# zhoubin-me/agent0

Hardware: AMD Instinct MI355X
Metric: env-frames/sec (learner FPS: transitions collected and saved to replay per second with the learner running, pre-frameskip) (higher is better)
Workload: dtype f32

## Files before the change

### agent0_amd/csrc/encoder_fused.hip

```cpp
#include "a0_internal.h"
#include "net_tables.h"
#include "operands.h"
#include "update_tail.h"

#include <cstdlib>
#include <type_traits>

typedef float a0_acc4 __attribute__((ext_vector_type(4)));

struct a0_fused_args {
    const uint8_t* frames; const int* slot; long long sample_stride; int chan_off;
    const float *wt1, *wt2, *wt3;
    const float *wx2, *wx3;
    const float *b1, *b2, *b3;
    float *act1, *act2, *act3;
    int B;
    int C, H, W, H1, W1, H2, W2, H3, W3;
    int off_act1, off_act2, off_end;
    int rp1, rp2;
};

A0_HD void a0_fused_set_wt(a0_fused_args& P, const float* wt, int C) {
    const a0_wt_layout T{C};
    P.wt1 = wt + T.conv1x(); P.wt2 = wt + T.conv2(); P.wt3 = wt + T.conv3(); P.wx2 = wt + T.conv2x(); P.wx3 = wt + T.conv3x();
// ... 405 lines not shown
        for (int i = 0; i < HB0; ++i)
            if (h * HB0 + i < MBT) {
#pragma unroll
                for (int t = 0; t < 3; ++t) a[slot][i][t] = *(const uint4*)(af.planes + rows[h * HB0 + i] + off + t * AFX::term);
            }
    };
    fetch(0, 0, af.step_off(wk));
    __builtin_amdgcn_s_waitcnt(0x0F70);
#pragma unroll 1
    for (int tb = 0; tb < NSTW; tb += R) {
#pragma unroll
        for (int u = 0; u < R; ++u) {
            const int st = wk + WK * (tb + u);
            const int off = af.step_off(st), offn = af.step_off(tb + u + 1 < NSTW ? st + WK : st);
#pragma unroll
            for (int h = 0; h < 2; ++h) {
                if (h == 0) fetch(1, 1, off);
                else fetch(0, 0, offn);
                __builtin_amdgcn_sched_barrier(0);
#pragma unroll
                for (int ta = 0; ta < 3; ++ta)
#pragma unroll
                    for (int tw = 0; tw < 3; ++tw)
#pragma unroll
                        for (int i = 0; i < HB0; ++i) {
                            if (ta + tw > ORD || h * HB0 + i >= MBT) continue;
                            const a0_u32x4 av = {a[h][i][ta].x, a[h][i][ta].y, a[h][i][ta].z, a[h][i][ta].w};
                            const a0_u32x4 bv = {ring.v[u][0][tw].x, ring.v[u][0][tw].y, ring.v[u][0][tw].z, ring.v[u][0][tw].w};
                            acc[h * HB0 + i] = __builtin_amdgcn_mfma_f32_16x16x32_bf16(__builtin_bit_cast(a0_bf16x8, bv), __builtin_bit_cast(a0_bf16x8, av), acc[h * HB0 + i], 0, 0, 0);
                        }
                __builtin_amdgcn_sched_barrier(0);
            }
            ring.fill(u);
            __builtin_amdgcn_sched_barrier(0);
        }
    }
    between();
    a0_acc4* x0 = (a0_acc4*)xch0;
    a0_acc4* x1 = (a0_acc4*)xch1;
    constexpr int P1 = (HB1 - 1) * 64 + 4 * LR;
    const int last = q * LR + r16;
    const int n0 = wn * 16 + 4 * q;
    float pe[EPI::PER_ELEM ? HB0 : 1][4];
    auto send = [&](auto mine) {
        constexpr int H = decltype(mine)::value;
        if constexpr (EPI::PER_ELEM) {
#pragma unroll
            for (int i = 0; i < (H == 0 ? HB0 : HB1); ++i) {
                const int m = (H * HB0 + i) * 16 + r16;
                const a0_f4 v = epi.pre_elem4(m < M ? m : M - 1, n0);
                pe[i][0] = v.x; pe[i][1] = v.y; pe[i][2] = v.z; pe[i][3] = v.w;
            }
        }
        if constexpr (H == 1) {
#pragma unroll
            for (int i = 0; i < HB0; ++i) x0[(wn * HB0 + i) * 64 + lane] = acc[i];
        } else {
#pragma unroll
            for (int i = 0; i < HB1; ++i) {
                if (i < HB1 - 1) x1[wn * P1 + i * 64 + lane] = acc[HB0 + i];
                else if (r16 < LR) x1[wn * P1 + (HB1 - 1) * 64 + last] = acc[HB0 + i];
            }
        }
    };
    auto recv = [&](auto mine) {
        constexpr int H = decltype(mine)::value;
#pragma unroll
        for (int i = 0; i < (H == 0 ? HB0 : HB1); ++i) {
            const int mb = H * HB0 + i;
            const int m = mb * 16 + r16;
            if constexpr (H == 0) acc[mb] += x0[(wn * HB0 + i) * 64 + lane];
            else {
                if (i < HB1 - 1) acc[mb] += x1[wn * P1 + i * 64 + lane];
                else if (r16 < LR) acc[mb] += x1[wn * P1 + (HB1 - 1) * 64 + last];
            }
            if (mb < MB && m < M) epi.emit_n4(m, n0, acc[mb], EPI::PER_ELEM ? pe[EPI::PER_ELEM ? i : 0] : nullptr);
        }
    };
    if (wk == 0) send(std::integral_constant<int, 0>{});
    else send(std::integral_constant<int, 1>{});
    __syncthreads();
    if (wk == 0) recv(std::integral_constant<int, 0>{});
    else recv(std::integral_constant<int, 1>{});
    __syncthreads();
}
constexpr int A0_P1X = 40, A0_P2X = 80;
constexpr int A0_RP1X = 20 * A0_P1X + 8;
constexpr int A0_RP2X = 9 * A0_P2X + 96;

constexpr int A0_R1 = 4, A0_R2 = 4, A0_R3 = 6;

template <int MBW1, int MBW2, int MBW3, int WC, bool X9, bool LOOP = false, int ORD = 4>
__global__ __launch_bounds__(A0_FUSED_THREADS) void a0_encoder_fused_kernel(a0_fused_args P);

constexpr int A0_X9_BIAS_OFF = 2 * 4 * 84 * 84 + 3 * 20 * A0_RP1X * 2;
constexpr int A0_RK2 = 2, A0_RK3 = 3;
constexpr int A0_X9_XCH0 = 3 * 9 * A0_RP2X * 2;
constexpr int A0_X9_XCH1 = A0_X9_BIAS_OFF + 160 * 4;
static_assert(A0_X9_XCH0 + 4 * 3 * 1024 <= 2 * 4 * 84 * 84, "conv2 exchange region 0 fits into the image");
constexpr int A0_X9_LDS_BYTES = A0_X9_XCH1 + 4 * (2 * 64 + 4) * 16;
static_assert(A0_X9_LDS_BYTES <= 160 * 1024, "LDS");
static_assert(A0_FUSED_WAVES == 8, "N-stationary stages: four waves along N, two along K");
typedef a0_wring9<64, 4, A0_RK2, 2> a0_ring2_t;
typedef a0_wring9<64, 4, A0_RK3, 2> a0_ring3_t;
template <int ORD, bool LOOP>
A0_D void a0_x9_conv23(const a0_fused_args& P, int b, unsigned char* smem, float* bias_lds, a0_wring1<A0_R1>& ring1, a0_ring2_t& ring2, a0_ring3_t& ring3) {
    const int obs_bytes = P.C * P.H * P.W;
    const int M2 = P.H2 * P.W2, M3 = P.H3 * P.W3;
    uint16_t* a1p = (uint16_t*)(smem + 2 * obs_bytes);
    constexpr int term1 = 20 * A0_RP1X, term2 = 9 * A0_RP2X;
    uint16_t* a2p = (uint16_t*)smem;
    typedef EpiFwdX<9, A0_P2X, A0_RP2X, term2> E2X;
    const AF2X<term1> f2{a1p, A0_RP1X, P.W2, A0_P1X};
    const E2X e2{bias_lds + 32, a2p, P.act2 ? P.act2 + (long long)b * M2 * 64 : nullptr, 64};
    const AF3X<term2> f3{a2p, A0_RP2X, P.W3, A0_P2X};
    const EpiFwdT e3{bias_lds + 96, P.act3 + (long long)b * M3 * 64, 64};
    a0_conv_stage_x9k<ORD, 64, 4, 6, A0_RK2, 1>(f2, M2, ring2, e2, (float*)(smem + A0_X9_XCH0), (float*)(smem + A0_X9_XCH1), [&] { ring3.prologue(); });
    a0_conv_stage_x9k<ORD, 64, 4, 4, A0_RK3, 16>(f3, M3, ring3, e3, (float*)a1p, (float*)a1p + 4 * 2 * 256, [&] { if (LOOP) ring1.prologue(); });
}

A0_D void a0_bytes16_to_img(uint16_t* img, int idx16, const uint4& v) {
    const uint32_t w[4] = {v.x, v.y, v.z, v.w};
    uint32_t o[8];
#pragma unroll
    for (int k = 0; k < 4; ++k) {
        const uint32_t f0 = __float_as_uint((float)(w[k] & 0xffu)), f1 = __float_as_uint((float)((w[k] >> 8) & 0xffu));
        const uint32_t f2 = __float_as_uint((float)((w[k] >> 16) & 0xffu)), f3 = __float_as_uint((float)(w[k] >> 24));
        o[2 * k] = __builtin_amdgcn_perm(f1, f0, 0x07060302u);
        o[2 * k + 1] = __builtin_amdgcn_perm(f3, f2, 0x07060302u);
    }
    ((uint4*)img)[2 * idx16] = uint4{o[0], o[1], o[2], o[3]};
    ((uint4*)img)[2 * idx16 + 1] = uint4{o[4], o[5], o[6], o[7]};
}

template <int ORD, bool LOOP>
A0_D void a0_encoder_fused_x9_body(const a0_fused_args& P, int bid, int nblk) {
    extern __shared__ __attribute__((aligned(16))) unsigned char smem[];
    uint16_t* img = (uint16_t*)smem;
    const int obs_bytes = P.C * P.H * P.W;
    const int M1 = P.H1 * P.W1;
    uint16_t* a1p = (uint16_t*)(smem + 2 * obs_bytes);
    constexpr int term1 = 20 * A0_RP1X;
    typedef EpiFwdX<20, A0_P1X, A0_RP1X, term1> E1X;
    a0_wring1<A0_R1> ring1;
    a0_ring2_t ring2;
    a0_ring3_t ring3;
    ring1.init(P.wt1, P.C);
    ring2.init(P.wx2, 512);
    ring3.init(P.wx3, 576);
    ring1.prologue();
    constexpr int MBW1X = (25 + A0_WMG1 - 1) / A0_WMG1;
    a0_pre<32, 2, MBW1X, E1X> pre1;
    float* bias_lds = (float*)(smem + A0_X9_BIAS_OFF);
    if (threadIdx.x < 160) bias_lds[threadIdx.x] = threadIdx.x < 32 ? P.b1[threadIdx.x] : threadIdx.x < 96 ? P.b2[threadIdx.x - 32] : P.b3[threadIdx.x - 96];
    for (int b = bid; b < P.B; b += nblk) {
        const long long s = P.slot ? (long long)P.slot[b] : (long long)b;
        const uint4* src = (const uint4*)(P.frames + s * P.sample_stride + P.chan_off);
        constexpr int TRIPS = 4;
        const int n16 = obs_bytes >> 4;
        for (int i0 = threadIdx.x; i0 < n16; i0 += TRIPS * A0_FUSED_THREADS) {
            uint4 v[TRIPS];
#pragma unroll
            for (int j = 0; j < TRIPS; ++j) {
                const int i = i0 + j * A0_FUSED_THREADS;
                v[j] = src[i < n16 ? i : n16 - 1];
            }
#pragma unroll
            for (int j = 0; j < TRIPS; ++j) {
                const int i = i0 + j * A0_FUSED_THREADS;
                a0_bytes16_to_img(img, i < n16 ? i : n16 - 1, v[j]);
            }
        }
        __syncthreads();
        const E1X e1{bias_lds, a1p, P.act1 ? P.act1 + (long long)b * M1 * 32 : nullptr, 32};
        const int wmg1 = __builtin_amdgcn_readfirstlane(threadIdx.x >> 6) / 2;
        if (MBW1X > 1 && wmg1 + (MBW1X - 1) * A0_WMG1 >= ((M1 + 15) >> 4))
            a0_conv1_stage<(MBW1X > 1 ? MBW1X - 1 : 1), A0_R1, 84>(img, P.H * P.W, P.W, P.W1, M1, ring1, e1, pre1, [&] { ring2.prologue(); });
        else
            a0_conv1_stage<MBW1X, A0_R1, 84>(img, P.H * P.W, P.W, P.W1, M1, ring1, e1, pre1, [&] { ring2.prologue(); });
        a0_x9_conv23<ORD, LOOP>(P, b, smem, bias_lds, ring1, ring2, ring3);
        if constexpr (!LOOP) break;
    }
}

#include "actor_tail.h"
struct a0_step_enc_args { const float *wt, *b1, *b2, *b3; float* act3; };
template <int ORD>
__global__ __launch_bounds__(A0_FUSED_THREADS) void a0_actor_dist_step_enc_kernel(a0_dtenv_args Q, a0_step_enc_args N) {
    __shared__ int s_chase_cell;
    extern __shared__ __attribute__((aligned(16))) unsigned char smem[];
    unsigned long long v_wt = (unsigned long long)N.wt, v_b1 = (unsigned long long)N.b1, v_b2 = (unsigned long long)N.b2, v_b3 = (unsigned long long)N.b3,
                       v_a3 = (unsigned long long)N.act3, v_obs = (unsigned long long)Q.obs_out;
    A0_TO_VGPR(v_wt); A0_TO_VGPR(v_b1); A0_TO_VGPR(v_b2); A0_TO_VGPR(v_b3); A0_TO_VGPR(v_a3); A0_TO_VGPR(v_obs);
    int v_E = Q.E;
    A0_TO_VGPR(v_E);
    a0_actor_dist_tail_env_body(Q, (float*)smem, &s_chase_cell);
    __syncthreads();
    auto uni = [](unsigned long long v) {
        return ((unsigned long long)(unsigned)__builtin_amdgcn_readfirstlane((int)(v >> 32)) << 32) | (unsigned long long)(unsigned)__builtin_amdgcn_readfirstlane((int)(v & 0xffffffffull));
    };
    const float* wt = (const float*)uni(v_wt);
    a0_fused_args P;
    P.frames = (const uint8_t*)uni(v_obs); P.slot = nullptr; P.sample_stride = 4 * 84 * 84; P.chan_off = 0;
    a0_fused_set_wt(P, wt, 4);
    P.b1 = (const float*)uni(v_b1); P.b2 = (const float*)uni(v_b2); P.b3 = (const float*)uni(v_b3);
    P.act1 = nullptr; P.act2 = nullptr; P.act3 = (float*)uni(v_a3); P.B = __builtin_amdgcn_readfirstlane(v_E);
    P.C = 4; P.H = 84; P.W = 84; P.H1 = 20; P.W1 = 20; P.H2 = 9; P.W2 = 9; P.H3 = 7; P.W3 = 7;
    P.off_act1 = 0; P.off_act2 = 0; P.off_end = 0; P.rp1 = 0; P.rp2 = 0;
    a0_encoder_fused_x9_body<ORD, false>(P, (int)blockIdx.x, (int)gridDim.x);
}

template <int MBW, class EPI, class Mid, class Between>
A0_D void a0_conv1_stage_split(const uint16_t* img, a0_wring1<A0_R1>& ring, const EPI& epi, bool first_before_mid, Mid&& mid, Between&& between) {
    static_assert(A0_R1 == 4 && EPI::TR, "ring of four steps, transposed accumulators");
    constexpr int HW = 84 * 84, W = 84, W1 = 20, M = 400, MB = 25;
// ... 186 lines not shown
        if (has_group()) {
#pragma unroll
            for (int c = 0; c < 4; ++c) row16[c * G16] = keep[c];
            const int nc = !chase ? 4 : (!term ? 3 : 0);
#pragma unroll
            for (int c = 0; c < 4; ++c)
                if (c < nc) { out16[c * G16] = keep[4 + c]; row16[(4 + c) * G16] = keep[4 + c]; }
        }
    };
    auto mid = [&] {
        if (wave != 0) early_stores();
        __syncthreads();
        if (chase) {
            if (has_group()) {
                uint32_t by, bx;
                a0_chase_pos(s_chase_cell, by, bx);
                const uint4 nw = new_group(by, bx);
                if (term) { put(0, nw); put(1, nw); put(2, nw); }
                put(3, nw);
            }
            __syncthreads();
        }
    };
    auto uni = [](unsigned long long v) {
        return ((unsigned long long)(unsigned)__builtin_amdgcn_readfirstlane((int)(v >> 32)) << 32) | (unsigned long long)(unsigned)__builtin_amdgcn_readfirstlane((int)(v & 0xffffffffull));
    };
    ring2.init((const float*)uni(v_wx2), 512);
    ring3.init((const float*)uni(v_wx3), 576);
    typedef EpiFwdX<20, A0_P1X, A0_RP1X, 20 * A0_RP1X> E1X;
    const E1X e1{bias_lds, a1p, nullptr, 32};
    constexpr int MBW1X = (25 + A0_WMG1 - 1) / A0_WMG1;
    const bool before = early && wave != 0;
    if (MBW1X > 1 && wave / 2 + (MBW1X - 1) * A0_WMG1 >= 25)
        a0_conv1_stage_split<(MBW1X > 1 ? MBW1X - 1 : 1)>(img, ring1, e1, before, mid, [&] { ring2.prologue(); });
    else
        a0_conv1_stage_split<MBW1X>(img, ring1, e1, before, mid, [&] { ring2.prologue(); });
    P.act3 = (float*)uni((unsigned long long)act3_v);
    a0_x9_conv23<ORD, false>(P, (int)e, smem, bias_lds, ring1, ring2, ring3);
}

template <int ORD>
__global__ __launch_bounds__(A0_FUSED_THREADS) void a0_actor_step_enc2_kernel(a0_qenv_args Q, a0_step_enc_args N) { a0_actor_step_enc2_body<ORD, TailScalar>(Q, N); }

static bool a0_fused_layout(int C, int H, int W, a0_fused_args& P, size_t& lds_bytes);
int a0_actor_dist_step_enc_launch(const a0_dtenv_args& Q, size_t tail_lds, const float* wt, const a0_encoder_weights* w, float* act3, hipStream_t st) {
    a0_fused_args P;
    size_t lds = 0;
    if (!wt || !w || !w->b1 || !w->b2 || !w->b3 || !act3 || !a0_fused_layout(4, 84, 84, P, lds)) return a0_fail(A0_EINVAL, "a0_actor_dist_tail_env_step_enc: bad encoder argument");
    if (P.H1 != 20 || P.W1 != 20 || P.H2 != 9 || P.W2 != 9 || P.H3 != 7 || P.W3 != 7) return a0_fail(A0_EINVAL, "a0_actor_dist_tail_env_step_enc: geometry");
    const a0_step_enc_args N{wt, w->b1, w->b2, w->b3, act3};
    lds = A0_X9_LDS_BYTES > tail_lds ? (size_t)A0_X9_LDS_BYTES : tail_lds;
    if (lds > 160 * 1024 - 64) return a0_fail(A0_EINVAL, "a0_actor_dist_tail_env_step_enc: head too wide for LDS");
    const int six = a0_x9_products_now() == 6;
    auto kern = six ? a0_actor_dist_step_enc_kernel<2> : a0_actor_dist_step_enc_kernel<4>;
    static size_t configured[2] = {0, 0};
    if (lds > configured[six]) {
        if (hipFuncSetAttribute((const void*)kern, hipFuncAttributeMaxDynamicSharedMemorySize, (int)lds) != hipSuccess)
            return a0_fail(A0_EINVAL, "a0_actor_dist_tail_env_step_enc: LDS");
        configured[six] = lds;
    }
    A0_LAUNCH_PROBED(A0_TAG_ACTOR_STEP_ENC, 2.0 * (400.0 * 32 * 256 + 81.0 * 64 * 512 + 49.0 * 64 * 576) * Q.E, kern, dim3(Q.E), dim3(A0_FUSED_THREADS), lds, st, Q, N);
    return a0_fail_hip((int)hipGetLastError(), "a0_actor_dist_tail_env_step_enc");
}
int a0_actor_step_enc_launch(const a0_qenv_args& Q, const float* wt, const a0_encoder_weights* w, float* act3, hipStream_t st) {
    a0_fused_args P;
    size_t lds = 0;
    if (!wt || !w || !w->b1 || !w->b2 || !w->b3 || !act3 || !a0_fused_layout(4, 84, 84, P, lds)) return a0_fail(A0_EINVAL, "a0_actor_qhead_env_step_enc: bad encoder argument");
    if (P.H1 != 20 || P.W1 != 20 || P.H2 != 9 || P.W2 != 9 || P.H3 != 7 || P.W3 != 7) return a0_fail(A0_EINVAL, "a0_actor_qhead_env_step_enc: geometry");
    const a0_step_enc_args N{wt, w->b1, w->b2, w->b3, act3};
    const size_t tail_lds = (size_t)(Q.A + (Q.dueling ? 1 : 0)) * 512 * sizeof(float);
    lds = A0_X9_LDS_BYTES > tail_lds ? (size_t)A0_X9_LDS_BYTES : tail_lds;
    const int six = a0_x9_products_now() == 6;
    auto kern = six ? a0_actor_step_enc2_kernel<2> : a0_actor_step_enc2_kernel<4>;
    static size_t configured[2] = {0, 0};
    if (lds > configured[six]) {
        if (hipFuncSetAttribute((const void*)kern, hipFuncAttributeMaxDynamicSharedMemorySize, (int)lds) != hipSuccess)
            return a0_fail(A0_EINVAL, "a0_actor_qhead_env_step_enc: LDS");
        configured[six] = lds;
    }
    A0_LAUNCH_PROBED(A0_TAG_ACTOR_STEP_ENC, 2.0 * (400.0 * 32 * 256 + 81.0 * 64 * 512 + 49.0 * 64 * 576) * Q.E, kern, dim3(Q.E), dim3(A0_FUSED_THREADS), lds, st, Q, N);
    return a0_fail_hip((int)hipGetLastError(), "a0_actor_qhead_env_step_enc");
}

struct a0_fused_multi_args { a0_fused_args p[3]; int first[4]; };
template <int ORD>
__global__ __launch_bounds__(A0_FUSED_THREADS) void a0_encoder_fused_multi_kernel(a0_fused_multi_args M) {
    const int bid = (int)blockIdx.x;
    const int k = bid >= M.first[2] ? 2 : (bid >= M.first[1] ? 1 : 0);
    a0_encoder_fused_x9_body<ORD, true>(M.p[k], bid - M.first[k], M.first[k + 1] - M.first[k]);
}

template <int MBW1, int MBW2, int MBW3, int WC, bool X9, bool LOOP, int ORD>
__global__ __launch_bounds__(A0_FUSED_THREADS) void a0_encoder_fused_kernel(a0_fused_args P) {
    if constexpr (X9) {
        static_assert(MBW1 == 7 && MBW2 == 3 && MBW3 == 2 && WC == 84, "the split-operand body is written for the 4 x 84 x 84 geometry");
        a0_encoder_fused_x9_body<ORD, LOOP>(P, (int)blockIdx.x, (int)gridDim.x);
        return;
    }
    extern __shared__ __attribute__((aligned(16))) unsigned char smem[];
    uint16_t* img = (uint16_t*)smem;
    float* fl = (float*)smem;
    float* act1 = fl + P.off_act1;
    float* act2 = fl + P.off_act2;
    const int obs_bytes = P.C * P.H * P.W;
    const int M1 = P.H1 * P.W1, M2 = P.H2 * P.W2, M3 = P.H3 * P.W3;
    a0_wring1<A0_R1> ring1;
    a0_wring<64, 4, A0_R2> ring2;
    a0_wring<64, 4, A0_R3> ring3;
    ring1.init(P.wt1, P.C);
    ring2.init(P.wt2, 512);
    ring3.init(P.wt3, 576);
    ring1.prologue();
    constexpr int OW1 = WC == 84 ? 20 : 0, OW2 = WC == 84 ? 9 : 0;
    a0_pre<32, 2, MBW1, EpiFwd<OW1>> pre1;
    a0_pre<64, 4, MBW2, EpiFwd<OW2>> pre2;
    a0_pre<64, 4, MBW3, EpiFwd<0>> pre3;
    pre1.load(EpiFwd<OW1>{P.b1, nullptr, 0, 0, 1, nullptr, 32}, M1);
    pre2.load(EpiFwd<OW2>{P.b2, nullptr, 0, 0, 1, nullptr, 64}, M2);
    pre3.load(EpiFwd<0>{P.b3, nullptr, 0, 0, 1, nullptr, 64}, M3);
    for (int b = blockIdx.x; b < P.B; b += gridDim.x) {
        const long long s = P.slot ? (long long)P.slot[b] : (long long)b;
        const uint4* src = (const uint4*)(P.frames + s * P.sample_stride + P.chan_off);
        constexpr int TRIPS = 4;
        const int n16 = obs_bytes >> 4;
        for (int i0 = threadIdx.x; i0 < n16; i0 += TRIPS * A0_FUSED_THREADS) {
            uint4 v[TRIPS];
#pragma unroll
            for (int j = 0; j < TRIPS; ++j) {
                const int i = i0 + j * A0_FUSED_THREADS;
                v[j] = src[i < n16 ? i : n16 - 1];
            }
#pragma unroll
            for (int j = 0; j < TRIPS; ++j) {
                const int i = i0 + j * A0_FUSED_THREADS;
                a0_bytes16_to_img(img, i < n16 ? i : n16 - 1, v[j]);
            }
        }
        __syncthreads();
        const EpiFwd<OW1> e1{P.b1, act1, A0_P1, P.rp1, P.W1, P.act1 ? P.act1 + (long long)b * M1 * 32 : nullptr, 32};
        const int wmg1 = __builtin_amdgcn_readfirstlane(threadIdx.x >> 6) / 2;
        if (MBW1 > 1 && wmg1 + (MBW1 - 1) * 4 >= ((M1 + 15) >> 4))
            a0_conv1_stage<(MBW1 > 1 ? MBW1 - 1 : 1), A0_R1, WC>(img, P.H * P.W, P.W, P.W1, M1, ring1, e1, pre1, [&] { ring2.prologue(); });
        else
            a0_conv1_stage<MBW1, A0_R1, WC>(img, P.H * P.W, P.W, P.W1, M1, ring1, e1, pre1, [&] { ring2.prologue(); });
        AF2 f2{act1, P.rp1, P.W2};
        const EpiFwd<OW2> e2{P.b2, act2, A0_P2, P.rp2, P.W2, P.act2 ? P.act2 + (long long)b * M2 * 64 : nullptr, 64};
        a0_conv_stage<64, 4, MBW2, 3, A0_R2>(f2, M2, 512, ring2, e2, pre2, [&] { ring3.prologue(); });
        AF3 f3{act2, P.rp2, P.W3};
        const EpiFwd<0> e3{P.b3, nullptr, 0, 0, 1, P.act3 + (long long)b * M3 * 64, 64};
        a0_conv_stage<64, 4, MBW3, 3, A0_R3>(f3, M3, 576, ring3, e3, pre3, [&] { ring1.prologue(); });
    }
}

struct a0_dgrad_args {
    const float *d3, *act1, *act2;
    float *d2, *d1;
    const float *wd3, *wd2;
    int B;
};
constexpr int A0_RPDA = 11 * A0_P2X + 96, A0_RPDB = 11 * A0_P2X + 48;
constexpr int A0_DTERMA = 11 * A0_RPDA, A0_DTERMB = 11 * A0_RPDB;
struct AFD3X {
    static constexpr int term = A0_DTERMA;
    const uint16_t* planes;
    A0_D int row(int m) const { const int oh = m / 9, ow = m - oh * 9; return oh * A0_RPDA + ow * A0_P2X; }
    A0_D int step_off(int st) const { const int tap = st >> 1; return (tap / 3) * A0_RPDA + (tap % 3) * A0_P2X + 32 * (st & 1); }
};
struct AFD2X {
    static constexpr int term = A0_DTERMB;
    const uint16_t* planes;
    A0_D int row(int m) const { const int oh = m / 10, ow = m - oh * 10; return oh * A0_RPDB + ow * A0_P2X; }
    A0_D int step_off(int st) const { const int cell = st >> 1; return (cell >> 1) * A0_RPDB + (cell & 1) * A0_P2X + 32 * (st & 1); }
};
struct EpiBwd3X {
    static constexpr bool PER_ELEM = true;
    static constexpr bool ROW4 = false;
    static constexpr bool TR = true;
    const float* mask; float* dst; uint16_t* planes;
    A0_D a0_f4 pre_elem4(int m, int n0) const { return *(const a0_f4*)(mask + (unsigned)(m * 64 + n0)); }
    A0_D void emit_n4(int m, int n0, const a0_acc4& acc, const float* pre) const {
        float v[4];
#pragma unroll
        for (int r = 0; r < 4; ++r) v[r] = pre[r] > 0.f ? acc[r] : 0.f;
        *(a0_f4*)(dst + (unsigned)(m * 64 + n0)) = a0_f4{v[0], v[1], v[2], v[3]};
        uint2 hi, mid, lo;
        a0_split4(v, hi, mid, lo);
        const int oh = m / 9, ow = m - oh * 9;
        uint16_t* d = planes + (oh + 1) * A0_RPDB + (ow + 1) * A0_P2X + n0;
        *(uint2*)d = hi; *(uint2*)(d + A0_DTERMB) = mid; *(uint2*)(d + 2 * A0_DTERMB) = lo;
    }
};
static_assert((A0_RPDB % 4) == 0 && (A0_DTERMB % 4) == 0 && (A0_P2X % 4) == 0, "8-byte aligned plane writes");
struct EpiBwdPair {
    static constexpr bool PER_ELEM = true;
    static constexpr bool ROW4 = false;
    static constexpr bool TR = true;
    const float* mask; float* dst; int p0;
    A0_D unsigned gi(int m, int n0) const {
        const int p = p0 + (n0 >> 5), oh = m / 10, ow = m - oh * 10;
        return (unsigned)(((oh * 2 + (p >> 1)) * 20 + ow * 2 + (p & 1)) * 32 + (n0 & 31));
    }
    A0_D a0_f4 pre_elem4(int m, int n0) const { return *(const a0_f4*)(mask + gi(m, n0)); }
    A0_D void emit_n4(int m, int n0, const a0_acc4& acc, const float* pre) const {
        *(a0_f4*)(dst + gi(m, n0)) = a0_f4{pre[0] > 0.f ? acc[0] : 0.f, pre[1] > 0.f ? acc[1] : 0.f, pre[2] > 0.f ? acc[2] : 0.f, pre[3] > 0.f ? acc[3] : 0.f};
    }
};
template <int ORD>
__global__ __launch_bounds__(A0_FUSED_THREADS) void a0_encoder_dgrad_fused_x9_kernel(a0_dgrad_args P) {
    extern __shared__ __attribute__((aligned(16))) unsigned char smem[];
    uint16_t* plA = (uint16_t*)smem;
    uint16_t* plB = plA + 3 * A0_DTERMA;
    for (int i = threadIdx.x; i < 3 * (A0_DTERMA + A0_DTERMB) / 2; i += A0_FUSED_THREADS) ((uint32_t*)smem)[i] = 0u;
    float* const xch0 = (float*)(smem + 3 * (A0_DTERMA + A0_DTERMB) * 2);
    float* const xch1 = xch0 + 4 * 4 * 256;
    const int lane = threadIdx.x & 63, wave = __builtin_amdgcn_readfirstlane(threadIdx.x >> 6), wn = wave & 3, wk = wave >> 2;
    a0_wring9<64, 4, 3, 2> ring3;
    a0_wring9<64, 4, 2, 2> ringq[2];
    ring3.init(P.wd3, 576);
    ring3.prologue();
    const uint4* const wq = (const uint4*)P.wd2 + (((wn & 1) * 16 + (lane & 15)) * 4 + (lane >> 4)) * 3 + (wn >> 1) * 3072 + wk * 384;
    __syncthreads();
    for (int b = blockIdx.x; b < P.B; b += gridDim.x) {
        const a0_f4* src = (const a0_f4*)(P.d3 + (long long)b * 49 * 64);
        for (int i = threadIdx.x; i < 49 * 16; i += A0_FUSED_THREADS) {
            const a0_f4 v = src[i];
            const int pos = i >> 4, c4 = (i & 15) * 4, h = pos / 7, w = pos - h * 7;
            const float x[4] = {v.x, v.y, v.z, v.w};
            uint2 hi, mid, lo;
            a0_split4(x, hi, mid, lo);
            uint16_t* d = plA + (h + 2) * A0_RPDA + (w + 2) * A0_P2X + c4;
            *(uint2*)(d) = hi; *(uint2*)(d + A0_DTERMA) = mid; *(uint2*)(d + 2 * A0_DTERMA) = lo;
        }
        __syncthreads();
        const AFD3X f3{plA};
        const AFD2X f2{plB};
        const EpiBwd3X e3{P.act2 + (long long)b * 81 * 64, P.d2 + (long long)b * 81 * 64, plB};
        const EpiBwdPair e2a{P.act1 + (long long)b * 400 * 32, P.d1 + (long long)b * 400 * 32, 0};
        const EpiBwdPair e2b{P.act1 + (long long)b * 400 * 32, P.d1 + (long long)b * 400 * 32, 2};
        a0_conv_stage_x9k<ORD, 64, 4, 6, 3, 1>(f3, 81, ring3, e3, xch0, xch1, [&] { ringq[0].init_at(wq, 4, 768); ringq[0].prologue(); });
        a0_conv_stage_x9k<ORD, 64, 4, 7, 2, 4>(f2, 100, ringq[0], e2a, xch0, xch1, [&] { ringq[1].init_at(wq + 2 * 3072, 4, 768); ringq[1].prologue(); });
        a0_conv_stage_x9k<ORD, 64, 4, 7, 2, 4>(f2, 100, ringq[1], e2b, xch0, xch1, [&] { ring3.prologue(); });
    }
}

__global__ void a0_conv_wt_kernel(const float* __restrict__ w1, const float* __restrict__ w2, const float* __restrict__ w3, float* __restrict__ wt, int K1,
                                  float* __restrict__ wt2, const int* __restrict__ state, int* __restrict__ commit) {
    const bool mirror = wt2 != nullptr && state[4] != 0;
    if (commit != nullptr && blockIdx.x == 0 && threadIdx.x == 0) { commit[1] = commit[5]; commit[0] = 0; }
    const a0_wt_layout T{K1 / 64};
    const int i = blockIdx.x * blockDim.x + threadIdx.x;
    if (i >= T.total()) return;
    uint32_t out = 0;
    if (i >= T.conv2() && i < T.conv2x()) {
        const bool c3 = i >= T.conv3();
        const int e = i - (c3 ? T.conv3() : T.conv2());
        const int j = e & 3, q = (e >> 2) & 3, n = (e >> 4) & 63, k = 16 * (e >> 10) + 4 * j + q;
        out = __float_as_uint(c3 ? w3[n * 576 + k] : w2[n * 512 + k]);
    } else {
        enum { CONV1, CONV2, CONV3, DGRAD3, DGRAD2 } seg;
        int e, N = 64, phase = 0;
        if (i < T.conv2()) { seg = CONV1; e = i; N = 32; }
        else if (i < T.conv3x()) { seg = CONV2; e = i - T.conv2x(); }
        else if (i < T.dgrad3x()) { seg = CONV3; e = i - T.conv3x(); }
        else if (i < T.dgrad2x()) { seg = DGRAD3; e = i - T.dgrad3x(); }
        else { seg = DGRAD2; e = i - T.dgrad2x(); phase = e / T.n_dgrad2x_phase; e -= phase * T.n_dgrad2x_phase; N = 32; }
        const int pair = e & 3, f = e >> 2, s = f % 3, q = (f / 3) & 3, n = (f / 12) % N, t = f / (12 * N);
        for (int h = 0; h < 2; ++h) {
            const int k = 32 * t + 8 * q + 2 * pair + h, cell = k >> 6, co = k & 63;
            float w;
            if (seg == CONV1) w = w1[n * K1 + k] / 255.0f;
            else if (seg == CONV2) w = w2[n * 512 + k];
            else if (seg == CONV3) w = w3[n * 576 + k];
            else if (seg == DGRAD3) {
                const int kh = 2 - cell / 3, kw = 2 - cell % 3;
                w = w3[co * 576 + (kh * 3 + kw) * 64 + n];
            } else {
                const int kh = (phase >> 1) + 2 * (1 - (cell >> 1)), kw = (phase & 1) + 2 * (1 - (cell & 1));
                w = w2[co * 512 + (kh * 4 + kw) * 32 + n];
            }
            out |= a0_bf16_term(w, s) << (16 * h);
        }
    }
    *(uint32_t*)(wt + i) = out;
    if (mirror) *(uint32_t*)(wt2 + i) = out;
}

extern "C" long long a0_net_conv_wt_floats(int C) { return a0_wt_layout{C}.total(); }

extern "C" int a0_net_conv_wt_refresh(const a0_encoder_weights* w, int C, float* wt, void* stream) {
    if (!w || !w->w1 || !w->w2 || !w->w3 || !wt || C < 1) return a0_fail(A0_EINVAL, "a0_net_conv_wt_refresh: bad argument");
    const long long n = a0_net_conv_wt_floats(C);
    hipLaunchKernelGGL(a0_conv_wt_kernel, dim3((unsigned)((n + 255) / 256)), dim3(256), 0, (hipStream_t)stream, w->w1, w->w2, w->w3, wt, C * 64, (float*)nullptr,
                       (const int*)nullptr, (int*)nullptr);
    return a0_fail_hip((int)hipGetLastError(), "a0_net_conv_wt_refresh");
}

extern "C" int a0_net_conv_wt_refresh_sync(const a0_encoder_weights* w, int C, float* wt, float* wt_target, const int* state, void* stream) {
    if (!w || !w->w1 || !w->w2 || !w->w3 || !wt || !wt_target || !state || C < 1) return a0_fail(A0_EINVAL, "a0_net_conv_wt_refresh_sync: bad argument");
    const long long n = a0_net_conv_wt_floats(C);
    hipLaunchKernelGGL(a0_conv_wt_kernel, dim3((unsigned)((n + 255) / 256)), dim3(256), 0, (hipStream_t)stream, w->w1, w->w2, w->w3, wt, C * 64, wt_target, state, (int*)nullptr);
    return a0_fail_hip((int)hipGetLastError(), "a0_net_conv_wt_refresh_sync");
}

int a0_conv_wt_refresh_commit(const a0_encoder_weights* w, int C, float* wt, float* wt_target, int* state, hipStream_t st) {
    if (!w || !w->w1 || !w->w2 || !w->w3) return a0_fail(A0_EINVAL, "a0_adam_step_sync_wt: encoder weights missing");
    const long long n = a0_net_conv_wt_floats(C);
    hipLaunchKernelGGL(a0_conv_wt_kernel, dim3((unsigned)((n + 255) / 256)), dim3(256), 0, st, w->w1, w->w2, w->w3, wt, C * 64, wt_target, (const int*)state, state);
    return a0_fail_hip((int)hipGetLastError(), "a0_adam_step_sync_wt");
}

static bool a0_fused_layout(int C, int H, int W, a0_fused_args& P, size_t& lds_bytes) {
    a0_net_core n;
    if (!a0_net_core_init(n, C, H, W)) return false;
    const int M1 = n.H1 * n.W1, M2 = n.H2 * n.W2, M3 = n.H3 * n.W3;
    if (M1 > 7 * 4 * 16 || M2 > 4 * 2 * 16 || M3 > 2 * 2 * 16) return false;
    if ((C * 2) % A0_R1 || (W & 3)) return false;
    const int obs_bytes = C * H * W;
    if (obs_bytes % 16) return false;
    P.C = C; P.H = H; P.W = W; P.H1 = n.H1; P.W1 = n.W1; P.H2 = n.H2; P.W2 = n.W2; P.H3 = n.H3; P.W3 = n.W3;
    P.rp1 = n.W1 * A0_P1;
    while ((P.rp1 - n.W2) & 15) ++P.rp1;
    P.rp2 = n.W2 * A0_P2;
    while ((P.rp2 - 2 * n.W3) & 31) ++P.rp2;
    P.off_act1 = obs_bytes / 2;
    P.off_act2 = P.off_act1 + ((n.H1 * P.rp1 + 3) & ~3);
    P.off_end = P.off_act2 + ((n.H2 * P.rp2 + 3) & ~3);
    lds_bytes = (size_t)P.off_end * 4;
    return lds_bytes <= 160 * 1024;
}

static bool a0_fused_fill(int C, int H, int W, const float* wt, const a0_encoder_weights* w, const a0_frames_arg* f, float* act1, float* act2, float* act3, int B,
                          a0_fused_args& P, size_t& lds_bytes) {
    if (!a0_fused_layout(C, H, W, P, lds_bytes)) return false;
    P.frames = f->frames; P.slot = f->slot; P.sample_stride = f->sample_stride; P.chan_off = f->chan_off;
    a0_fused_set_wt(P, wt, C);
    P.b1 = w->b1; P.b2 = w->b2; P.b3 = w->b3;
    P.act1 = act1; P.act2 = act2; P.act3 = act3; P.B = B;
    return true;
}

extern "C" int a0_net_encoder_fused_supported(int C, int H, int W) {
    a0_fused_args P; size_t lds;
    return a0_fused_layout(C, H, W, P, lds) ? 1 : 0;
}

extern "C" int a0_net_encoder_fwd_fused(int C, int H, int W, const float* wt, const a0_encoder_weights* w, const a0_frames_arg* f, int B,
                                        float* act1, float* act2, float* act3, void* stream) {
    A0_TRY
    if (!wt || !w || !w->b1 || !w->b2 || !w->b3 || !f || !f->frames || !act3 || B < 1) return a0_fail(A0_EINVAL, "a0_net_encoder_fwd_fused: bad argument");
    a0_fused_args P;
    size_t lds = 0;
    if (!a0_fused_fill(C, H, W, wt, w, f, act1, act2, act3, B, P, lds)) return a0_fail(A0_EINVAL, "a0_net_encoder_fwd_fused: observation shape not supported by the fused kernel");
    if ((f->sample_stride % 16) || (f->chan_off % 16) || (((uintptr_t)f->frames) % 16)) return a0_fail(A0_EINVAL, "a0_net_encoder_fwd_fused: frames must be 16-byte aligned");
    const int mb1 = (P.H1 * P.W1 + 15) / 16, mb2 = (P.H2 * P.W2 + 15) / 16, mb3 = (P.H3 * P.W3 + 15) / 16;
    const bool standard = ((mb1 + 3) / 4 == 7) && ((mb2 + 1) / 2 == 3) && ((mb3 + 1) / 2 == 2) && W == 84;
    const bool x9 = standard && H == 84 && C == 4;
    int which = x9 ? 2 : (standard ? 1 : 0);
    if (x9) lds = A0_X9_LDS_BYTES;
    static_assert(3 * 9 * A0_RP2X * 2 <= 2 * 4 * 84 * 84, "the act2 term planes fit into the dead image");
    const int gridx = (which == 2 && B > 256) ? 256 : B;
    if (which == 2 && gridx < B) which = 3;
    static size_t configured[6] = {0, 0, 0, 0, 0, 0};
    const int six = a0_x9_products_now() == 6;
    if (six && which >= 2) which += 2;
    typedef void (*a0_enc_kern)(a0_fused_args);
    const a0_enc_kern fn = which == 5 ? a0_encoder_fused_kernel<7, 3, 2, 84, true, true, 2> : which == 4 ? a0_encoder_fused_kernel<7, 3, 2, 84, true, false, 2>
                         : which == 3 ? a0_encoder_fused_kernel<7, 3, 2, 84, true, true> : which == 2 ? a0_encoder_fused_kernel<7, 3, 2, 84, true>
                         : which == 1 ? a0_encoder_fused_kernel<7, 3, 2, 84, false> : a0_encoder_fused_kernel<7, 4, 2, 0, false>;
    if (lds > configured[which]) {
        A0_HIP_THROW(hipFuncSetAttribute((const void*)fn, hipFuncAttributeMaxDynamicSharedMemorySize, (int)lds));
        configured[which] = lds;
    }
    const double per_obs = 2.0 * ((double)P.H1 * P.W1 * 32 * (P.C * 64) + (double)P.H2 * P.W2 * 64 * 512 + (double)P.H3 * P.W3 * 64 * 576);
    A0_LAUNCH_PROBED(A0_TAG_ENCODER_FUSED, per_obs * B, fn, dim3((which == 3 || which == 5) ? gridx : B), dim3(A0_FUSED_THREADS), lds, (hipStream_t)stream, P);
    A0_HIP_THROW(hipGetLastError());
    return A0_OK;
    A0_CATCH
}

extern "C" int a0_net_encoder_fwd_fused_multi(int C, int H, int W, int n, const a0_encoder_pass* pass, void* stream) {
    A0_TRY
    if (n < 1 || n > 3 || !pass) return a0_fail(A0_EINVAL, "a0_net_encoder_fwd_fused_multi: 1 to 3 passes");
    if (!(C == 4 && H == 84 && W == 84)) return a0_fail(A0_EINVAL, "a0_net_encoder_fwd_fused_multi: 4 x 84 x 84 observations on the split-operand kernel only");
    a0_fused_multi_args M;
    size_t lds = 0;
    long long total = 0;
    for (int i = 0; i < n; ++i) {
        const a0_encoder_pass& q = pass[i];
        if (!q.wt || !q.w || !q.w->b1 || !q.w->b2 || !q.w->b3 || !q.f || !q.f->frames || !q.act3 || q.B < 1) return a0_fail(A0_EINVAL, "a0_net_encoder_fwd_fused_multi: bad pass");
        if ((q.f->sample_stride % 16) || (q.f->chan_off % 16) || (((uintptr_t)q.f->frames) % 16)) return a0_fail(A0_EINVAL, "a0_net_encoder_fwd_fused_multi: frames must be 16-byte aligned");
        if (!a0_fused_fill(C, H, W, q.wt, q.w, q.f, q.act1, q.act2, q.act3, q.B, M.p[i], lds))
            return a0_fail(A0_EINVAL, "a0_net_encoder_fwd_fused_multi: observation shape");
        total += q.B;
    }
    for (int i = n; i < 3; ++i) M.p[i] = M.p[0];
    int grid = (int)(total < 256 ? total : 256), used = 0;
    if (grid < n) grid = n;
    for (int i = 0; i < n; ++i) {
        M.first[i] = used;
        int share = (i == n - 1) ? grid - used : (int)((long long)grid * pass[i].B / total);
        if (share < 1) share = 1;
        if (share > pass[i].B) share = pass[i].B;
        used += share;
    }
    for (int i = n; i <= 3; ++i) M.first[i] = 0x7fffffff;
    M.first[n] = used;
    lds = A0_X9_LDS_BYTES;
    const int six = a0_x9_products_now() == 6;
    auto kern = six ? a0_encoder_fused_multi_kernel<2> : a0_encoder_fused_multi_kernel<4>;
    static bool configured[2] = {false, false};
    if (!configured[six]) {
        A0_HIP_THROW(hipFuncSetAttribute((const void*)kern, hipFuncAttributeMaxDynamicSharedMemorySize, (int)lds));
        configured[six] = true;
    }
    const a0_fused_args& P0 = M.p[0];
    const double per_obs = 2.0 * ((double)P0.H1 * P0.W1 * 32 * (P0.C * 64) + (double)P0.H2 * P0.W2 * 64 * 512 + (double)P0.H3 * P0.W3 * 64 * 576);
    A0_LAUNCH_PROBED(A0_TAG_ENCODER_FUSED, per_obs * (double)total, kern, dim3(used), dim3(A0_FUSED_THREADS), lds, (hipStream_t)stream, M);
    A0_HIP_THROW(hipGetLastError());
    return A0_OK;
    A0_CATCH
}

extern "C" int a0_net_encoder_dgrad_fused_supported(int C, int H, int W) { return (C >= 1 && H == 84 && W == 84) ? 1 : 0; }

extern "C" int a0_net_encoder_dgrad_fused(int C, int H, int W, const float* wt, const float* d3, const float* act1, const float* act2, int B, float* d2,
                                          float* d1, void* stream) {
    A0_TRY
    if (!wt || !d3 || !act1 || !act2 || !d2 || !d1 || B < 1) return a0_fail(A0_EINVAL, "a0_net_encoder_dgrad_fused: bad argument");
    if (!a0_net_encoder_dgrad_fused_supported(C, H, W)) return a0_fail(A0_EINVAL, "a0_net_encoder_dgrad_fused: 84x84 observations only");
    a0_dgrad_args P;
    P.d3 = d3; P.act1 = act1; P.act2 = act2; P.d2 = d2; P.d1 = d1; P.B = B;
    P.wd3 = wt + a0_wt_layout{C}.dgrad3x(); P.wd2 = wt + a0_wt_layout{C}.dgrad2x();
    const size_t lds = (size_t)3 * (A0_DTERMA + A0_DTERMB) * 2 + (4 * 4 + 4 * 3) * 1024;
    static bool configured[2] = {false, false};
    const int six = a0_x9_products_now() == 6;
    auto fn = six ? a0_encoder_dgrad_fused_x9_kernel<2> : a0_encoder_dgrad_fused_x9_kernel<4>;
    if (!configured[six]) {
        A0_HIP_THROW(hipFuncSetAttribute((const void*)fn, hipFuncAttributeMaxDynamicSharedMemorySize, (int)lds));
        configured[six] = true;
    }
    const int gridx = B > 256 ? 256 : B;
    A0_LAUNCH_PROBED(A0_TAG_ENCODER_DGRAD_FUSED, 2.0 * (81.0 * 64 * 576 + 400.0 * 32 * 256) * B, fn, dim3(gridx), dim3(A0_FUSED_THREADS), lds, (hipStream_t)stream, P);
    A0_HIP_THROW(hipGetLastError());
    return A0_OK;
    A0_CATCH
}
```

Measured before the change: 2.481 million.

## Flatten multi-pass encoder scheduling and merge dgrad conv2 phases into one stage

```diff
diff --git a/agent0_amd/csrc/encoder_fused.hip b/agent0_amd/csrc/encoder_fused.hip
--- a/agent0_amd/csrc/encoder_fused.hip
+++ b/agent0_amd/csrc/encoder_fused.hip
@@ -511,6 +511,90 @@
     __syncthreads();
     if (wk == 0) recv(std::integral_constant<int, 0>{});
     else recv(std::integral_constant<int, 1>{});
+    __syncthreads();
+}
+template <int ORD, int MBT, class AFX, class EPI, class Between>
+A0_D void a0_conv_stage_x9n(const AFX& af, int M, a0_wring9<128, 8, 2, 1>& ring, const EPI& epi, Between&& between) {
+    constexpr int R = 2, HB0 = (MBT + 1) / 2, HB1 = MBT / 2;
+    static_assert(HB1 >= 1 && EPI::TR && EPI::PER_ELEM, "tile shape");
+    const int tid = threadIdx.x, lane = tid & 63;
+    const int wave = __builtin_amdgcn_readfirstlane(tid >> 6);
+    const int q = lane >> 4, r16 = lane & 15;
+    const int NST = ring.nst;
+    int rows[MBT];
+#pragma unroll
+    for (int i = 0; i < MBT; ++i) {
+        const int m = i * 16 + r16;
+        rows[i] = af.row(m < M ? m : 0) + 8 * q;
+    }
+    a0_acc4 acc[R][MBT];
+#pragma unroll
+    for (int u = 0; u < R; ++u)
+#pragma unroll
+        for (int i = 0; i < MBT; ++i) acc[u][i] = a0_acc4{0.f, 0.f, 0.f, 0.f};
+    uint4 a[2][HB0][3];
+    auto fetch = [&](int slot, int h, int off) {
+#pragma unroll
+        for (int i = 0; i < HB0; ++i)
+            if (h * HB0 + i < MBT) {
+#pragma unroll
+                for (int t = 0; t < 3; ++t) a[slot][i][t] = *(const uint4*)(af.planes + rows[h * HB0 + i] + off + t * AFX::term);
+            }
+    };
+    const int n0 = wave * 16 + 4 * q;
+    float pe[MBT][4];
+    auto turn = [&](int tb, auto last) {
+        constexpr bool LAST = decltype(last)::value;
+#pragma unroll
+        for (int u = 0; u < R; ++u) {
+            const int st = tb + u;
+            const int off = af.step_off(st), offn = af.step_off(st + 1);
+#pragma unroll
+            for (int h = 0; h < 2; ++h) {
+                if (h == 0) fetch(1, 1, off);
+                else if (!LAST || u + 1 < R) fetch(0, 0, offn);
+                else {
+#pragma unroll
+                    for (int i = 0; i < MBT; ++i) {
+                        const int m = i * 16 + r16;
+                        const a0_f4 v = epi.pre_elem4(m < M ? m : M - 1, n0);
+                        pe[i][0] = v.x; pe[i][1] = v.y; pe[i][2] = v.z; pe[i][3] = v.w;
+                    }
+                }
+                __builtin_amdgcn_sched_barrier(0);
+#pragma unroll
+                for (int ta = 0; ta < 3; ++ta)
+#pragma unroll
+                    for (int tw = 0; tw < 3; ++tw)
+#pragma unroll
+                        for (int i = 0; i < HB0; ++i) {
+                            if (ta + tw > ORD || h * HB0 + i >= MBT) continue;
+                            const a0_u32x4 av = {a[h][i][ta].x, a[h][i][ta].y, a[h][i][ta].z, a[h][i][ta].w};
+                            const a0_u32x4 bv = {ring.v[u][0][tw].x, ring.v[u][0][tw].y, ring.v[u][0][tw].z, ring.v[u][0][tw].w};
+                            acc[u][h * HB0 + i] = __builtin_amdgcn_mfma_f32_16x16x32_bf16(__builtin_bit_cast(a0_bf16x8, bv), __builtin_bit_cast(a0_bf16x8, av), acc[u][h * HB0 + i], 0, 0, 0);
+                        }
+                __builtin_amdgcn_sched_barrier(0);
+            }
+            if (!LAST) ring.fill(u);
+            __builtin_amdgcn_sched_barrier(0);
+        }
+    };
+    fetch(0, 0, af.step_off(0));
+    __builtin_amdgcn_s_waitcnt(0x0F70);
+#pragma unroll 1
+    for (int tb = 0; tb < NST - R; tb += R) turn(tb, std::false_type{});
+    turn(NST - R, std::true_type{});
+#pragma unroll
+    for (int i = 0; i < MBT; ++i) acc[0][i] += acc[1][i];
+    between();
+#pragma unroll
+    for (int i = 0; i < MBT; ++i) epi.apply4(acc[0][i], pe[i]);
+    __builtin_amdgcn_sched_barrier(0);
+#pragma unroll
+    for (int i = 0; i < MBT; ++i) {
+        const int m = i * 16 + r16;
+        if (m < M) epi.store_n4(m, n0, acc[0][i]);
+    }
     __syncthreads();
 }
 constexpr int A0_P1X = 40, A0_P2X = 80;
@@ -560,6 +644,43 @@
     }
     ((uint4*)img)[2 * idx16] = uint4{o[0], o[1], o[2], o[3]};
     ((uint4*)img)[2 * idx16 + 1] = uint4{o[4], o[5], o[6], o[7]};
+}
+
+constexpr int A0_MBW1X = (25 + A0_WMG1 - 1) / A0_WMG1;
+typedef EpiFwdX<20, A0_P1X, A0_RP1X, 20 * A0_RP1X> a0_e1x_t;
+A0_D void a0_x9_obs_conv1(const a0_fused_args& P, int b, unsigned char* smem, float* bias_lds, a0_wring1<A0_R1>& ring1, a0_ring2_t& ring2) {
+    uint16_t* img = (uint16_t*)smem;
+    const int obs_bytes = P.C * P.H * P.W;
+    const int M1 = P.H1 * P.W1;
+    uint16_t* a1p = (uint16_t*)(smem + 2 * obs_bytes);
+    a0_pre<32, 2, A0_MBW1X, a0_e1x_t> pre1;
+    const long long s = P.slot ? (long long)P.slot[b] : (long long)b;
+    const uint4* src = (const uint4*)(P.frames + s * P.sample_stride + P.chan_off);
+    constexpr int TRIPS = 4;
+    const int n16 = obs_bytes >> 4;
+    for (int i0 = threadIdx.x; i0 < n16; i0 += TRIPS * A0_FUSED_THREADS) {
+        uint4 v[TRIPS];
+#pragma unroll
+        for (int j = 0; j < TRIPS; ++j) {
+            const int i = i0 + j * A0_FUSED_THREADS;
+            v[j] = src[i < n16 ? i : n16 - 1];
+        }
+#pragma unroll
+        for (int j = 0; j < TRIPS; ++j) {
+            const int i = i0 + j * A0_FUSED_THREADS;
+            a0_bytes16_to_img(img, i < n16 ? i : n16 - 1, v[j]);
+        }
+    }
+    __syncthreads();
+    const a0_e1x_t e1{bias_lds, a1p, P.act1 ? P.act1 + (long long)b * M1 * 32 : nullptr, 32};
+    const int wmg1 = __builtin_amdgcn_readfirstlane(threadIdx.x >> 6) / 2;
+    if (A0_MBW1X > 1 && wmg1 + (A0_MBW1X - 1) * A0_WMG1 >= ((M1 + 15) >> 4))
+        a0_conv1_stage<(A0_MBW1X > 1 ? A0_MBW1X - 1 : 1), A0_R1, 84>(img, P.H * P.W, P.W, P.W1, M1, ring1, e1, pre1, [&] { ring2.prologue(); });
+    else
+        a0_conv1_stage<A0_MBW1X, A0_R1, 84>(img, P.H * P.W, P.W, P.W1, M1, ring1, e1, pre1, [&] { ring2.prologue(); });
+}
+A0_D void a0_x9_bias_to_lds(const a0_fused_args& P, float* bias_lds) {
+    if (threadIdx.x < 160) bias_lds[threadIdx.x] = threadIdx.x < 32 ? P.b1[threadIdx.x] : threadIdx.x < 96 ? P.b2[threadIdx.x - 32] : P.b3[threadIdx.x - 96];
 }
 
 template <int ORD, bool LOOP>
@@ -912,12 +1033,41 @@
     return a0_fail_hip((int)hipGetLastError(), "a0_actor_qhead_env_step_enc");
 }
 
-struct a0_fused_multi_args { a0_fused_args p[3]; int first[4]; };
+struct a0_fused_multi_args { a0_fused_args p[3]; int end[3]; };
 template <int ORD>
 __global__ __launch_bounds__(A0_FUSED_THREADS) void a0_encoder_fused_multi_kernel(a0_fused_multi_args M) {
-    const int bid = (int)blockIdx.x;
-    const int k = bid >= M.first[2] ? 2 : (bid >= M.first[1] ? 1 : 0);
-    a0_encoder_fused_x9_body<ORD, true>(M.p[k], bid - M.first[k], M.first[k + 1] - M.first[k]);
+    extern __shared__ __attribute__((aligned(16))) unsigned char smem[];
+    const int G = (int)gridDim.x, total = M.end[2], w = (int)blockIdx.x;
+    const int nj = (total - w + G - 1) / G;
+    const int dj = (w & 1) ? -1 : 1;
+    int j = (w & 1) ? nj - 1 : 0;
+    int it = w + j * G;
+    int k = (it >= M.end[0] ? 1 : 0) + (it >= M.end[1] ? 1 : 0);
+    a0_wring1<A0_R1> ring1;
+    a0_ring2_t ring2;
+    a0_ring3_t ring3;
+    ring1.init(M.p[k].wt1, 4);
+    ring1.prologue();
+    float* bias_lds = (float*)(smem + A0_X9_BIAS_OFF);
+    bool fresh = true;
+    for (int i = 0;;) {
+        const a0_fused_args& P = M.p[k];
+        if (fresh) {
+            ring2.init(P.wx2, 512);
+            ring3.init(P.wx3, 576);
+            a0_x9_bias_to_lds(P, bias_lds);
+        }
+        const int b = it - (k == 0 ? 0 : M.end[k - 1]);
+        a0_x9_obs_conv1(P, b, smem, bias_lds, ring1, ring2);
+        const int jn = j + dj;
+        const int nx = i + 1 < nj ? w + jn * G : it;
+        const int kn = (nx >= M.end[0] ? 1 : 0) + (nx >= M.end[1] ? 1 : 0);
+        ring1.init(M.p[kn].wt1, 4);
+        a0_x9_conv23<ORD, true>(P, b, smem, bias_lds, ring1, ring2, ring3);
+        if (++i == nj) break;
+        fresh = kn != k;
+        k = kn; j = jn; it = nx;
+    }
 }
 
 template <int MBW1, int MBW2, int MBW3, int WC, bool X9, bool LOOP, int ORD>
@@ -1021,34 +1171,37 @@
     }
 };
 static_assert((A0_RPDB % 4) == 0 && (A0_DTERMB % 4) == 0 && (A0_P2X % 4) == 0, "8-byte aligned plane writes");
-struct EpiBwdPair {
+struct EpiBwdPhases {
     static constexpr bool PER_ELEM = true;
     static constexpr bool ROW4 = false;
     static constexpr bool TR = true;
-    const float* mask; float* dst; int p0;
+    const float* mask; float* dst;
     A0_D unsigned gi(int m, int n0) const {
-        const int p = p0 + (n0 >> 5), oh = m / 10, ow = m - oh * 10;
+        const int p = n0 >> 5, oh = m / 10, ow = m - oh * 10;
         return (unsigned)(((oh * 2 + (p >> 1)) * 20 + ow * 2 + (p & 1)) * 32 + (n0 & 31));
     }
     A0_D a0_f4 pre_elem4(int m, int n0) const { return *(const a0_f4*)(mask + gi(m, n0)); }
-    A0_D void emit_n4(int m, int n0, const a0_acc4& acc, const float* pre) const {
-        *(a0_f4*)(dst + gi(m, n0)) = a0_f4{pre[0] > 0.f ? acc[0] : 0.f, pre[1] > 0.f ? acc[1] : 0.f, pre[2] > 0.f ? acc[2] : 0.f, pre[3] > 0.f ? acc[3] : 0.f};
-    }
-};
+    A0_D void apply4(a0_acc4& acc, const float* pre) const {
+#pragma unroll
+        for (int r = 0; r < 4; ++r) acc[r] = pre[r] > 0.f ? acc[r] : 0.f;
+    }
+    A0_D void store_n4(int m, int n0, const a0_acc4& acc) const { *(a0_f4*)(dst + gi(m, n0)) = a0_f4{acc[0], acc[1], acc[2], acc[3]}; }
+};
+static_assert((3 * (A0_DTERMA + A0_DTERMB) * 2) % 16 == 0, "the padded images are zeroed 16 bytes at a time");
 template <int ORD>
 __global__ __launch_bounds__(A0_FUSED_THREADS) void a0_encoder_dgrad_fused_x9_kernel(a0_dgrad_args P) {
     extern __shared__ __attribute__((aligned(16))) unsigned char smem[];
     uint16_t* plA = (uint16_t*)smem;
     uint16_t* plB = plA + 3 * A0_DTERMA;
-    for (int i = threadIdx.x; i < 3 * (A0_DTERMA + A0_DTERMB) / 2; i += A0_FUSED_THREADS) ((uint32_t*)smem)[i] = 0u;
+    for (int i = threadIdx.x; i < 3 * (A0_DTERMA + A0_DTERMB) / 8; i += A0_FUSED_THREADS) ((uint4*)smem)[i] = uint4{0u, 0u, 0u, 0u};
     float* const xch0 = (float*)(smem + 3 * (A0_DTERMA + A0_DTERMB) * 2);
     float* const xch1 = xch0 + 4 * 4 * 256;
-    const int lane = threadIdx.x & 63, wave = __builtin_amdgcn_readfirstlane(threadIdx.x >> 6), wn = wave & 3, wk = wave >> 2;
+    const int lane = threadIdx.x & 63, wave = __builtin_amdgcn_readfirstlane(threadIdx.x >> 6);
     a0_wring9<64, 4, 3, 2> ring3;
-    a0_wring9<64, 4, 2, 2> ringq[2];
+    a0_wring9<128, 8, 2, 1> ringq;
     ring3.init(P.wd3, 576);
     ring3.prologue();
-    const uint4* const wq = (const uint4*)P.wd2 + (((wn & 1) * 16 + (lane & 15)) * 4 + (lane >> 4)) * 3 + (wn >> 1) * 3072 + wk * 384;
+    ringq.init_at((const uint4*)P.wd2 + (((wave & 1) * 16 + (lane & 15)) * 4 + (lane >> 4)) * 3 + (wave >> 1) * 3072, 8, 384);
     __syncthreads();
     for (int b = blockIdx.x; b < P.B; b += gridDim.x) {
         const a0_f4* src = (const a0_f4*)(P.d3 + (long long)b * 49 * 64);
@@ -1065,11 +1218,9 @@
         const AFD3X f3{plA};
         const AFD2X f2{plB};
         const EpiBwd3X e3{P.act2 + (long long)b * 81 * 64, P.d2 + (long long)b * 81 * 64, plB};
-        const EpiBwdPair e2a{P.act1 + (long long)b * 400 * 32, P.d1 + (long long)b * 400 * 32, 0};
-        const EpiBwdPair e2b{P.act1 + (long long)b * 400 * 32, P.d1 + (long long)b * 400 * 32, 2};
-        a0_conv_stage_x9k<ORD, 64, 4, 6, 3, 1>(f3, 81, ring3, e3, xch0, xch1, [&] { ringq[0].init_at(wq, 4, 768); ringq[0].prologue(); });
-        a0_conv_stage_x9k<ORD, 64, 4, 7, 2, 4>(f2, 100, ringq[0], e2a, xch0, xch1, [&] { ringq[1].init_at(wq + 2 * 3072, 4, 768); ringq[1].prologue(); });
-        a0_conv_stage_x9k<ORD, 64, 4, 7, 2, 4>(f2, 100, ringq[1], e2b, xch0, xch1, [&] { ring3.prologue(); });
+        const EpiBwdPhases e2{P.act1 + (long long)b * 400 * 32, P.d1 + (long long)b * 400 * 32};
+        a0_conv_stage_x9k<ORD, 64, 4, 6, 3, 1>(f3, 81, ring3, e3, xch0, xch1, [&] { ringq.prologue(); });
+        a0_conv_stage_x9n<ORD, 7>(f2, 100, ringq, e2, [&] { ring3.prologue(); });
     }
 }
 
@@ -1224,17 +1375,13 @@
         total += q.B;
     }
     for (int i = n; i < 3; ++i) M.p[i] = M.p[0];
-    int grid = (int)(total < 256 ? total : 256), used = 0;
-    if (grid < n) grid = n;
-    for (int i = 0; i < n; ++i) {
-        M.first[i] = used;
-        int share = (i == n - 1) ? grid - used : (int)((long long)grid * pass[i].B / total);
-        if (share < 1) share = 1;
-        if (share > pass[i].B) share = pass[i].B;
-        used += share;
-    }
-    for (int i = n; i <= 3; ++i) M.first[i] = 0x7fffffff;
-    M.first[n] = used;
+    if (total > 0x3fffffff) return a0_fail(A0_EINVAL, "a0_net_encoder_fwd_fused_multi: too many observations");
+    int used = 0;
+    for (int i = 0; i < 3; ++i) {
+        if (i < n) used += pass[i].B;
+        M.end[i] = used;
+    }
+    used = used < 256 ? used : 256;
     lds = A0_X9_LDS_BYTES;
     const int six = a0_x9_products_now() == 6;
     auto kern = six ? a0_encoder_fused_multi_kernel<2> : a0_encoder_fused_multi_kernel<4>;
```

Result: no change. 2.503 million, median of 6 (+0.9%).
